# UWQuickstep/quickstep

Hardware: AMD Instinct MI355X
Metric: probe+aggregate rows/s at TPC-H SF100 (Q1,Q3) (higher is better)
Workload: dtype i32 keys / f64 sums

## Files before the change

### quickstep_amd/capi.py

```python
import ctypes as C
import os

import torch

from . import types as T

_HERE = os.path.dirname(os.path.abspath(__file__))
LIB_PATH = os.environ.get("QSX_LIB_PATH") or os.path.join(_HERE, "lib", "libqsx.so")


class QsxError(RuntimeError):
    def __init__(self, status, where):
        self.status = status
        msg = _lib.qsx_status_string(status).decode()
        detail = _lib.qsx_last_error().decode()
        super().__init__(f"{where}: {msg} ({status})" + (f" — {detail}" if detail and status in (T.ERR_HIP, T.ERR_COMM) else ""))


def _load():
    if not os.path.exists(LIB_PATH):
        raise ImportError(
            f"{LIB_PATH} is missing: build it with `python -c 'import __graft_entry__ as g; g.build()'` "
            "(or make -C quickstep_amd/csrc). There is no CPU fallback for the HIP execution kernel.")
    return C.CDLL(LIB_PATH)
# ... 1078 lines not shown
        _check(_lib.qsx_agg_state_export_bytes(self._h, C.byref(v), _stream(stream)), "qsx_agg_state_export_bytes")
        return v.value

    def export(self, device, stream=None):
        nbytes = self.export_bytes(stream)
        out = torch.empty(nbytes // 8, dtype=torch.int64, device=device)
        _check(_lib.qsx_agg_state_export(self._h, _ptr(out), nbytes, _stream(stream)), "qsx_agg_state_export")
        return out

    def image_layout(self):
        dense, header, per_col, ncols = C.c_int(), C.c_int64(), C.c_int64(), C.c_int()
        kinds = (C.c_int32 * 32)()
        _check(_lib.qsx_agg_state_image_layout(self._h, C.byref(dense), C.byref(header), C.byref(per_col), C.byref(ncols), kinds, 32),
               "qsx_agg_state_image_layout")
        return bool(dense.value), header.value, per_col.value, [int(kinds[i]) for i in range(ncols.value)]

    def import_merge(self, image, stream=None):
        _check(_lib.qsx_agg_state_import_merge(self._h, _ptr(image), image.numel() * image.element_size(), _stream(stream)),
               "qsx_agg_state_import_merge")

    def num_groups(self, stream=None):
        v = C.c_int64()
        _check(_lib.qsx_agg_num_groups(self._h, C.byref(v), _stream(stream)), "qsx_agg_num_groups")
        return v.value

    def finalize(self, device, partition=0, num_partitions=1, capacity=None, stream=None):
        cfg = self.config
        if capacity is None:
            capacity = max(self.num_groups(stream), 1)
        keys = []
        for k in range(cfg.num_keys):
            w = cfg.column_width[cfg.key_column[k]]
            dt = {1: torch.uint8, 2: torch.int16, 4: torch.int32, 8: torch.int64}[w]
            keys.append(torch.zeros(capacity, dtype=dt, device=device))
        vals, nulls = [], []
        for a in range(cfg.num_aggs):
            dt = getattr(torch, T.agg_output_dtype(cfg, a))
            vals.append(torch.zeros(capacity, dtype=dt, device=device))
            nulls.append(torch.zeros(capacity, dtype=torch.uint8, device=device))
        groups = torch.zeros(1, dtype=torch.int64, device=device)
        _check(_lib.qsx_agg_finalize(self._h, partition, num_partitions, _ptr_array(keys), _ptr_array(vals),
                                     _ptr_array(nulls), capacity, _ptr(groups), _stream(stream)), "qsx_agg_finalize")
        return keys, vals, nulls, groups


class LipFilter:
    def __init__(self, kind, cardinality, min_value=0, is_anti=False):
        h = C.c_void_p()
        _check(_lib.qsx_lip_filter_create(kind, cardinality, min_value, 1 if is_anti else 0, C.byref(h)),
               "qsx_lip_filter_create")
        self._h = h

    def close(self):
        if self._h is not None:
            _lib.qsx_lip_filter_destroy(self._h)
            self._h = None

    def __del__(self):
        try:
            self.close()
        except Exception:
            pass

    def build(self, keys, filter_bitmap=None, stream=None):
        _check(_lib.qsx_lip_build(self._h, qsx_type_of(keys), _ptr(keys), keys.numel(), _ptr(filter_bitmap),
                                  _stream(stream)), "qsx_lip_build")

    def build_from_table(self, table, num_new_keys=-1, stream=None):
        rc = _lib.qsx_lip_build_from_join_table(self._h, table._h, num_new_keys, _stream(stream))
        if rc == T.ERR_UNSUPPORTED:
            return False
        _check(rc, "qsx_lip_build_from_join_table")
        return True
# ... 168 lines not shown
```

### quickstep_amd/csrc/aggregate.hip

```cpp

#include "agg_common.hpp"
#include "agg_translate.hpp"
#include "agg_hash_update.hpp"
#include "agg_factored.hpp"
#include "agg_shapes.hpp"
#include "agg_stream.hpp"
#include "agg_family.hpp"
#include "agg_pieces.hpp"
#include "agg_jit.hpp"
#include "comm.hpp"
#include "partition.hpp"
#include "scan.hpp"

#include <atomic>
#include <cstdlib>
#include <map>
#include <mutex>
#include <shared_mutex>
#include <vector>

namespace qsx {

struct ColKinds {
  int kind[QSX_MAX_AGGS + 1];
// ... 48 lines not shown
    }
  }
}

__global__ __launch_bounds__(kABlock) void init_log_kernel(unsigned long long *__restrict__ log, int stride,
                                                          unsigned long long count, const unsigned int *__restrict__ count_dev,
                                                          unsigned int log_cap, ColKinds kinds) {
  if (count_dev != nullptr) count = *count_dev < log_cap ? *count_dev : log_cap;
  const unsigned long long words = count * stride;
  for (unsigned long long i = static_cast<unsigned long long>(blockIdx.x) * kABlock + threadIdx.x; i < words;
       i += static_cast<unsigned long long>(gridDim.x) * kABlock) {
    const int w = static_cast<int>(i % stride);
    log[i] = w == 0 ? kEmptyCode : static_cast<unsigned long long>(acc_identity(kinds.kind[w - 1]));
  }
}

__global__ __launch_bounds__(kABlock) void drain_log_kernel(const unsigned long long *__restrict__ records, unsigned int count,
                                                           int stride, int num_cols, ColKinds kinds, HashTableView g) {
  for (unsigned int r = blockIdx.x * kABlock + threadIdx.x; r < count; r += gridDim.x * kABlock) {
    const unsigned long long *rec = records + static_cast<unsigned long long>(r) * stride;
    const unsigned long long gs = global_find_or_insert(g, rec[0]);
    if (gs == ~0ull) continue;
    for (int col = 0; col < num_cols; ++col) global_add(g, col, gs, rec[1 + col], kinds.kind[col]);
  }
}

__global__ void publish_control_kernel(const unsigned long long *__restrict__ control, unsigned long long *host_slot,
                                       unsigned long long seq) {
  if (threadIdx.x != 0) return;
  __hip_atomic_store(&host_slot[0], control[0], __ATOMIC_RELAXED, __HIP_MEMORY_SCOPE_SYSTEM);
  __hip_atomic_store(&host_slot[1], control[3], __ATOMIC_RELAXED, __HIP_MEMORY_SCOPE_SYSTEM);
  __hip_atomic_store(&host_slot[2], control[1], __ATOMIC_RELAXED, __HIP_MEMORY_SCOPE_SYSTEM);
  __hip_atomic_store(&host_slot[3], seq, __ATOMIC_RELEASE, __HIP_MEMORY_SCOPE_SYSTEM);
}


__device__ __forceinline__ double avg_quotient(double s, double c) {
  const double q = s / c;
  if (!isfinite(q) || fabs(q) >= 2.2250738585072014e-308) return q;
  double best = q, best_r = fabs(fma(-q, c, s));
  const double around[2] = {nextafter(q, -INFINITY), nextafter(q, INFINITY)};
  for (const double x : around) {
    const double r = fabs(fma(-x, c, s));
    if (r < best_r || (r == best_r && (__double_as_longlong(x) & 1) == 0)) {
      best = x;
      best_r = r;
    }
  }
  return best;
}

__device__ __forceinline__ void write_values(const FinalizeDesc &f, const unsigned long long *states,
                                             unsigned long long col_stride, unsigned long long idx,
                                             int count_col, bool empty_group, long long out_row) {
  const long long cnt = count_col >= 0 ? static_cast<long long>(states[static_cast<unsigned long long>(count_col) * col_stride + idx]) : 0;
  for (int a = 0; a < f.num_aggs; ++a) {
    bool is_null = false;
    const bool has_nn = f.nn_col[a] >= 0;
    const long long seen = has_nn ? static_cast<long long>(states[static_cast<unsigned long long>(f.nn_col[a]) * col_stride + idx]) : cnt;
    if (f.fn[a] == QSX_AGG_COUNT_STAR) {
      static_cast<long long *>(f.out_vals[a])[out_row] = cnt;
    } else if (f.fn[a] == QSX_AGG_COUNT) {
      static_cast<long long *>(f.out_vals[a])[out_row] = seen;
    } else {
      const unsigned long long raw = states[static_cast<unsigned long long>(f.sum_col[a]) * col_stride + idx];
      if (f.fn[a] == QSX_AGG_SUM) {
// ... 35 lines not shown

__device__ __forceinline__ void write_keys_from_code(const FinalizeDesc &f, unsigned long long code, long long out_row,
                                                     const unsigned long long *states = nullptr, unsigned long long stride = 0,
                                                     unsigned long long slot = 0) {
  for (int k = 0; k < f.num_keys; ++k) {
    const unsigned long long v = group_key_word(f, code, states, stride, slot, f.key_word[k]) >> f.key_shift[k];
    switch (f.key_width[k]) {
      case 1: static_cast<uint8_t *>(f.out_keys[k])[out_row] = static_cast<uint8_t>(v); break;
      case 2: static_cast<uint16_t *>(f.out_keys[k])[out_row] = static_cast<uint16_t>(v); break;
      case 4: static_cast<uint32_t *>(f.out_keys[k])[out_row] = static_cast<uint32_t>(v); break;
      default: static_cast<unsigned long long *>(f.out_keys[k])[out_row] = v; break;
    }
  }
}

__device__ __forceinline__ unsigned long long reference_scalar_hash(int type, unsigned long long bits) {
  switch (type) {
    case QSX_INT: return bits & 0xFFFFFFFFull;
    case QSX_FLOAT: return (bits & 0xFFFFFFFFull) == 0x80000000ull ? 0ull : (bits & 0xFFFFFFFFull);
    case QSX_DOUBLE: return bits == 0x8000000000000000ull ? 0ull : bits;
    default: return bits;
  }
}
__device__ __forceinline__ unsigned long long reference_combine(unsigned long long a, unsigned long long b) {
  const unsigned long long kMul = 0x9ddfea08eb382d69ull;
  unsigned long long x = (a ^ b) * kMul;
  x ^= (x >> 47);
  unsigned long long y = (b ^ x) * kMul;
  y ^= (y >> 47);
  y *= kMul;
  return y;
}

__global__ __launch_bounds__(kABlock) void finalize_hash_kernel(HashTableView g, FinalizeDesc f,
                                                               int partition, int num_partitions,
                                                               int partition_by_hash, long long capacity,
                                                               unsigned long long *__restrict__ out_groups) {
  const unsigned long long stride = g.cap + 1;
  const unsigned long long total = g.cap + 1;
  const unsigned long long rounded = (total + kWave - 1) / kWave * kWave;
  for (unsigned long long i = static_cast<unsigned long long>(blockIdx.x) * kABlock + threadIdx.x;
       i < rounded; i += static_cast<unsigned long long>(gridDim.x) * kABlock) {
    bool emit = false;
    unsigned long long code = kEmptyCode;
    if (i < total) {
      code = i == g.cap ? kEmptyCode : g.keys[i];
      const unsigned long long cnt = g.states[i];
      emit = (i == g.cap) ? (cnt != 0) : (code != kEmptyCode);
      if (emit && partition_by_hash) {
        unsigned long long h = 0;
        for (int k = 0; k < f.num_keys; ++k) {
          unsigned long long bits = group_key_word(f, code, g.states, stride, i, f.key_word[k]) >> f.key_shift[k];
          if (f.key_width[k] < 8) bits &= (1ull << (8 * f.key_width[k])) - 1;
          const unsigned long long hk = reference_scalar_hash(f.key_type[k], bits);
          h = k == 0 ? hk : reference_combine(h, hk);
        }
        emit = static_cast<int>(h % static_cast<unsigned long long>(num_partitions)) == partition;
      }
    }
    const uint64_t m = __ballot(emit);
    if (m == 0) continue;
    const int leader = __ffsll(static_cast<long long>(m)) - 1;
    unsigned long long base = 0;
    if (lane_id() == leader) base = atomicAdd(out_groups, static_cast<unsigned long long>(__popcll(m)));
    base = __shfl(base, leader, kWave);
    if (!emit) continue;
    const long long out_row = static_cast<long long>(base) + rank_below(m);
    if (out_row >= capacity) continue;
    write_keys_from_code(f, code, out_row, g.states, stride, i);
    write_values(f, g.states, stride, i, 0, false, out_row);
  }
}

constexpr int kExprRows = 2;
struct ExprProgram {
  const void *cols[QSX_MAX_COLUMNS];
  int types[QSX_MAX_COLUMNS];
  int num_instrs;
  DevInstr instrs[QSX_MAX_INSTRS];
  double consts[QSX_MAX_CONSTS];
  DevOperand result;
};
static_assert(sizeof(ExprProgram) % 4 == 0, "store_struct_kernel copies words");
__device__ __forceinline__ void expr_operand(const ExprProgram &p, const DevOperand &o, const Temps<kExprRows> &t, const int64_t (&row)[kExprRows],
                                             double (&out)[kExprRows]) {
  switch (o.kind) {
    case QSX_OPD_COLUMN: {
      const void *col = as_global(p.cols[o.index]);
#pragma unroll
      for (int v = 0; v < kExprRows; ++v) {
        switch (p.types[o.index]) {
          case QSX_INT: out[v] = static_cast<double>(static_cast<const int32_t *>(col)[row[v]]); break;
          case QSX_LONG: out[v] = static_cast<double>(static_cast<const long long *>(col)[row[v]]); break;
          case QSX_FLOAT: out[v] = static_cast<double>(static_cast<const float *>(col)[row[v]]); break;
          default: out[v] = static_cast<const double *>(col)[row[v]]; break;
        }
      }
      break;
    }
    case QSX_OPD_CONST:
#pragma unroll
      for (int v = 0; v < kExprRows; ++v) out[v] = p.consts[o.index];
      break;
    default:
// ... 1505 lines not shown
  }
  if (err == hipSuccess && fill_identities(st, nullptr) != QSX_OK) err = hipErrorUnknown;
  if (err == hipSuccess) err = hipDeviceSynchronize();
  if (err != hipSuccess) {
    set_last_error("qsx_agg_state_create", err);
    (void)device_free(st->image); (void)device_free(st->control); (void)device_free(st->tile_counts); (void)device_free(st->tile_offsets);
    (void)device_free(st->log);
    (void)device_free(st->dir_entries); (void)device_free(st->dir_codes); (void)device_free(st->dir_words); (void)device_free(st->dir_ngids);
    published_slots().give(st->published);
    delete st;
    return err == hipErrorOutOfMemory ? QSX_ERR_OUT_OF_MEMORY : QSX_ERR_HIP;
  }
  *out = st;
  return QSX_OK;
}

int qsx_agg_state_destroy(qsx_agg_state_t *st) {
  if (st == nullptr) return QSX_OK;
  (void)synchronize_owner_device(st->image);
  (void)device_free_idle(st->image);
  (void)device_free_idle(st->control);
  (void)device_free_idle(st->tile_counts);
  (void)device_free_idle(st->tile_offsets);
  (void)device_free_idle(st->log);
  (void)device_free_idle(st->dir_entries);
  (void)device_free_idle(st->dir_codes);
  (void)device_free_idle(st->dir_words);
  (void)device_free_idle(st->dir_ngids);
  published_slots().give(st->published);
  delete st;
  return QSX_OK;
}

int qsx_agg_state_clear(qsx_agg_state_t *st, qsx_stream_t stream) {
  QSX_REQUIRE_DEVICE();
  if (st == nullptr) return QSX_ERR_INVALID_ARGUMENT;
  hipStream_t s = as_stream(stream);
  std::unique_lock<std::shared_mutex> lock(st->table_mutex);
  if (st->growable) {
    int rc = init_log(st, st->log, 0, reinterpret_cast<const unsigned int *>(st->control + 3), s);
    if (rc != QSX_OK) return rc;
    __atomic_store_n(&st->published[0], 0ull, __ATOMIC_RELEASE);
    __atomic_store_n(&st->published[1], 0ull, __ATOMIC_RELEASE);
  }
  if (st->dir_gids != 0) {
    QSX_HIP_TRY(hipMemsetAsync(st->dir_entries, 0xFF, st->dir_cap * 8 * st->dir_entry_words, s));
    QSX_HIP_TRY(hipMemsetAsync(st->dir_ngids, 0, 16, s));
  }
  if (st->dense) {
    QSX_HIP_TRY(hipMemsetAsync(st->image, 0, st->image_bytes, s));
  } else {
    QSX_HIP_TRY(hipMemsetAsync(st->image, 0xFF, sizeof(unsigned long long) * (st->cap + 1), s));
    QSX_HIP_TRY(hipMemsetAsync(st->image + (st->cap + 1), 0,
                               sizeof(unsigned long long) * (st->cap + 1) * st->num_cols, s));
  }
  QSX_HIP_TRY(hipMemsetAsync(st->control, 0, 8 * sizeof(unsigned long long), s));
  return fill_identities(st, s);
}

static void decide_dense_families(qsx_agg_state *st, const void *key_col, int64_t rows, hipStream_t s) {
  if (st->dense_families.load() != 0) return;
  DevConfig dev = st->dev;
  plan_tile(dev, st->used_columns, kDirBlock, false);
  const DenseLdsGeometry geo = dense_lds_geometry(st->config.num_entries, st->num_sums, static_cast<size_t>(dev.tile_bytes), true);
  if (geo.entries == 0 || geo.ranges == 1) {
    st->dense_families.store(1);
    return;
  }
  const int key_col_index = st->dev.key_column[0];
  const int sample = static_cast<int>(std::min<int64_t>(rows, 256 * 1024));
  if (key_col == nullptr || st->dev.code_width[key_col_index] != 0 || sample < 4096) {
// ... 1569 lines not shown
    switch (o.kind) {
      case QSX_OPD_COLUMN: return types[o.index] == QSX_INT;
      case QSX_OPD_CONST: return consts[o.index] >= INT32_MIN && consts[o.index] <= INT32_MAX;
      default: return temp_is_int[o.index];
    }
  };
  for (int k = 0; k < num_instrs; ++k) {
    const qsx_expr_instr_t &in = instrs[k];
    if (in.op < QSX_EX_ADD || in.op > QSX_EX_IDIV || in.dst < 0 || in.dst >= QSX_MAX_TEMPS || !valid(in.a) || !valid(in.b)) {
      return QSX_ERR_INVALID_ARGUMENT;
    }
    prog.instrs[k].op = in.op & 3;
    prog.instrs[k].dst = in.dst;
    prog.instrs[k].a = DevOperand{in.a.kind, in.a.index};
    prog.instrs[k].b = DevOperand{in.b.kind, in.b.index};
    prog.narrow[k] = is_int(in.a) && is_int(in.b) ? 1 : 0;
    temp_is_int[in.dst] = prog.narrow[k] != 0;
    defined |= 1 << in.dst;
  }
  if (!valid(result)) return QSX_ERR_INVALID_ARGUMENT;
  prog.result = DevOperand{result.kind, result.index};
  for (int k = 0; k < QSX_MAX_CONSTS; ++k) prog.consts[k] = consts != nullptr ? consts[k] : 0;
  if (n == 0) return QSX_OK;
  hipStream_t s = as_stream(stream);
  IntExprProgram *slot = device_slot<IntExprProgram>(s);
  if (slot == nullptr) return QSX_ERR_OUT_OF_MEMORY;
  hipLaunchKernelGGL(store_struct_kernel<IntExprProgram>, dim3(1), dim3(64), 0, s, prog, slot);
  QSX_CHECK_LAUNCH();
  hipLaunchKernelGGL(eval_expression_long_kernel, dim3(grid_for(n, kABlock * 4)), dim3(kABlock), 0, s, slot, n, out_width, out_dev);
  QSX_CHECK_LAUNCH();
  return QSX_OK;
}

int qsx_agg_finalize(qsx_agg_state_t *st, int partition, int num_partitions, void *const *out_key_cols,
                     void *const *out_val_cols, uint8_t *const *out_null_cols, int64_t capacity,
                     int64_t *out_groups_dev, qsx_stream_t stream) {
  QSX_REQUIRE_DEVICE();
  if (st == nullptr || out_groups_dev == nullptr || num_partitions < 1 || partition < 0 ||
      partition >= num_partitions || capacity < 0 || out_val_cols == nullptr) {
    return QSX_ERR_INVALID_ARGUMENT;
  }
  hipStream_t s = as_stream(stream);
  int rc = settle(st, s);
  if (rc != QSX_OK) return rc;
  std::shared_lock<std::shared_mutex> lock(st->table_mutex);
  FinalizeDesc f = st->fin;
  for (int k = 0; k < f.num_keys; ++k) {
    if (out_key_cols == nullptr || out_key_cols[k] == nullptr) return QSX_ERR_INVALID_ARGUMENT;
    f.out_keys[k] = out_key_cols[k];
  }
  for (int a = 0; a < f.num_aggs; ++a) {
    f.out_vals[a] = out_val_cols[a];
    f.out_nulls[a] = out_null_cols != nullptr ? out_null_cols[a] : nullptr;
  }
  unsigned long long *out_groups = reinterpret_cast<unsigned long long *>(out_groups_dev);
  QSX_HIP_TRY(hipMemsetAsync(out_groups_dev, 0, sizeof(int64_t), s));
  f.collision = reinterpret_cast<int *>(st->control + 4);
  switch (st->config.strategy) {
    case QSX_AGG_SINGLE_STATE:
      if (partition != 0) return QSX_OK;
      if (capacity < 1) return QSX_ERR_CAPACITY;
      hipLaunchKernelGGL(finalize_single_kernel, dim3(1), dim3(64), 0, s, st->hash_view(), f, out_groups);
      break;
    case QSX_AGG_COMPACT_KEY:
      if (partition != 0) return QSX_OK;
      hipLaunchKernelGGL(finalize_hash_kernel, dim3(grid_for(st->cap + 1, kABlock)), dim3(kABlock), 0, s,
                         st->hash_view(), f, 0, 1, 0, static_cast<long long>(capacity), out_groups);
      break;
    case QSX_AGG_GENERIC:
      hipLaunchKernelGGL(finalize_hash_kernel, dim3(grid_for(st->cap + 1, kABlock)), dim3(kABlock), 0, s,
                         st->hash_view(), f, partition, num_partitions, 1, static_cast<long long>(capacity),
                         out_groups);
      break;
    default: {
      const DenseRange range = dense_partition_range(st->config.num_entries, num_partitions, partition);
      const long long begin = range.begin, end = range.end;
      if (begin >= end) return QSX_OK;
      const long long first_word = range.first_word;
      const long long num_words = range.last_word - first_word;
      const long long num_tiles = (num_words + kDenseTileWords - 1) / kDenseTileWords;
      const DenseView d = st->dense_view();
      CallScratch scratch(s);
      const size_t counts_bytes = sizeof(int32_t) * static_cast<size_t>(num_tiles + 1), offsets_bytes = sizeof(int64_t) * static_cast<size_t>(num_tiles + 2);
      const int rc_scratch = scratch.reserve(CallScratch::padded(counts_bytes) + CallScratch::padded(offsets_bytes));
      if (rc_scratch != QSX_OK) return rc_scratch;
      int32_t *tile_counts = static_cast<int32_t *>(scratch.take(counts_bytes));
      int64_t *tile_offsets = static_cast<int64_t *>(scratch.take(offsets_bytes));
      hipLaunchKernelGGL(dense_tile_count_kernel, dim3(grid_for(num_tiles, kABlock / kWave)), dim3(kABlock), 0, s,
                         d.exist, first_word, num_words, begin, end, num_tiles, tile_counts);
      QSX_CHECK_LAUNCH();
      hipLaunchKernelGGL(tile_scan_kernel, dim3(1), dim3(1024), 0, s, tile_counts,
                         static_cast<int64_t>(num_tiles), tile_offsets, out_groups_dev);
      QSX_CHECK_LAUNCH();
      hipLaunchKernelGGL(finalize_dense_kernel, dim3(grid_for(num_tiles, kABlock / kWave)), dim3(kABlock), 0, s,
                         d, f, first_word, num_words, begin, end, num_tiles, tile_offsets,
                         static_cast<long long>(capacity));
      break;
    }
  }
  QSX_CHECK_LAUNCH();
  if (f.wide_words != 0) {
    hipLaunchKernelGGL(report_collision_kernel, dim3(1), dim3(64), 0, s, f.collision, out_groups);
    QSX_CHECK_LAUNCH();
  }
  return QSX_OK;
}

}
```

### quickstep_amd/csrc/join.hip

```cpp

#include "common.hpp"
#include "join_dense.hpp"
#include "join_lds.hpp"
#include "scan.hpp"

#include <atomic>
#include <cstdlib>
#include <vector>
#include <mutex>
#include <shared_mutex>
#include <type_traits>

namespace qsx {

constexpr int kJBlock = 256;
constexpr uint64_t kEmpty64 = ~0ull;
constexpr uint32_t kEmptyTid = 0xFFFFFFFFu;

struct alignas(16) LongEntry {
  int64_t key;
  uint32_t tid;
  uint32_t pad;
};

// ... 219 lines not shown
  for (int64_t i = static_cast<int64_t>(blockIdx.x) * kJBlock + threadIdx.x; i < cap;
       i += static_cast<int64_t>(gridDim.x) * kJBlock) {
    if (is_long) {
      const LongEntry e = static_cast<const LongEntry *>(src.slots)[i];
      if (e.tid != kEmptyTid) insert_entry(dst, e.key, e.tid);
    } else {
      const uint64_t e = static_cast<const uint64_t *>(src.slots)[i];
      if (e != kEmpty64) {
        insert_entry(dst, static_cast<int32_t>(static_cast<uint32_t>(e)), static_cast<uint32_t>(e >> 32));
      }
    }
  }
}

__global__ __launch_bounds__(kJBlock) void compact_build_kernel(TableView t, uint32_t *__restrict__ cslots, unsigned char *__restrict__ cfp) {
  const uint64_t s = static_cast<uint64_t>(blockIdx.x) * kJBlock + threadIdx.x;
  if (s >= t.num_slots()) return;
  unsigned char f = 0;
  uint32_t packed = 0xFFFFFFFFu;
  if (t.fp[s] != 0) {
    const uint64_t e = static_cast<const uint64_t *>(t.slots)[s];
    const CompactId id = compact_id(static_cast<int32_t>(static_cast<uint32_t>(e)), t.buckets);
    if (id.bucket == static_cast<uint32_t>(s / kBucketSlots)) {
      f = static_cast<unsigned char>(id.fp);
      packed = (id.low << 24) | (static_cast<uint32_t>(e >> 32) & 0xFFFFFFu);
    } else {
      f = 0xFFu;
    }
  }
  cfp[s] = f;
  cslots[s] = packed;
}

__global__ __launch_bounds__(kJBlock) void dense_pack_kernel(const uint32_t *__restrict__ head, uint64_t range, unsigned char *__restrict__ head3) {
  for (uint64_t i = static_cast<uint64_t>(blockIdx.x) * kJBlock + threadIdx.x; i < range; i += static_cast<uint64_t>(gridDim.x) * kJBlock) {
    const uint32_t w = head[i];
    const uint32_t packed = (w & 0x7FFFFFu) | ((w & kChainBit) >> 8);
    head3[i * 3] = static_cast<unsigned char>(packed);
    head3[i * 3 + 1] = static_cast<unsigned char>(packed >> 8);
    head3[i * 3 + 2] = static_cast<unsigned char>(packed >> 16);
  }
}

__global__ __launch_bounds__(kJBlock) void dense_build_from_slots_kernel(int is_long, TableView src, DenseTableView d) {
  const int64_t cap = static_cast<int64_t>(src.num_slots());
  for (int64_t i = static_cast<int64_t>(blockIdx.x) * kJBlock + threadIdx.x; i < cap;
       i += static_cast<int64_t>(gridDim.x) * kJBlock) {
    int64_t key;
    uint32_t tid;
    if (is_long) {
      const LongEntry e = static_cast<const LongEntry *>(src.slots)[i];
      if (e.tid == kEmptyTid) continue;
      key = e.key;
      tid = e.tid;
    } else {
      const uint64_t e = static_cast<const uint64_t *>(src.slots)[i];
      if (e == kEmpty64) continue;
      key = static_cast<int32_t>(static_cast<uint32_t>(e));
      tid = static_cast<uint32_t>(e >> 32);
    }
    const uint64_t idx = dense_index(d, key);
    if (idx == ~0ull) {
      atomicExch(d.error, 1);
      continue;
    }
    const uint32_t old = atomicCAS(&d.head[idx], 0u, tid + 1u);
    if (old != 0u) {
      const unsigned int e = atomicAdd(d.ov_count, 1u);
      if (e >= d.ov_capacity) {
        atomicExch(d.error, 2);
        continue;
      }
      d.ov[e].x = tid;
      d.ov[e].y = atomicExch(&d.head[idx], kChainBit | e);
// ... 754 lines not shown
  return join_key_pack_blocks_impl(ncols, types, num_blocks, block_rows, block_cols, block_code_widths, block_dictionaries, out_dev, out_exact, stream);
}

static int destroy_table(qsx_join_table_t *t, bool wait_for_device) {
  if (t == nullptr) return QSX_OK;
  if (wait_for_device) {
    (void)synchronize_owner_device(t->slots != nullptr ? static_cast<const void *>(t->slots) : static_cast<const void *>(t->head));
  }
  if (t->shadow != nullptr) (void)destroy_table(t->shadow, wait_for_device);
  (void)device_free_idle(t->slots);
  (void)device_free_idle(t->head);
  (void)device_free_idle(t->head3);
  (void)device_free_idle(t->compact);
  (void)device_free_idle(t->cover);
  if (t->pack_event != nullptr) (void)hipEventDestroy(t->pack_event);
  if (t->seal_event != nullptr) (void)hipEventDestroy(t->seal_event);
  for (auto &m : t->marks) {
    if (m.second != nullptr) (void)hipEventDestroy(m.second);
  }
  if (t->control_host != nullptr) (void)hipHostFree(t->control_host);
  (void)device_free_idle(t->ov);
  (void)device_free_idle(t->entries_dev);
  delete t;
  return QSX_OK;
}
int qsx_join_table_destroy(qsx_join_table_t *t) { return destroy_table(t, true); }
int qsx_join_table_release(qsx_join_table_t *t) { return destroy_table(t, false); }

int qsx_join_table_clear(qsx_join_table_t *t, qsx_stream_t stream) {
  QSX_REQUIRE_DEVICE();
  if (t == nullptr) return QSX_ERR_INVALID_ARGUMENT;
  std::unique_lock<std::shared_mutex> lock(t->mutex);
  if (t->dense) {
    QSX_HIP_TRY(hipMemsetAsync(t->head, 0, t->range * sizeof(uint32_t), as_stream(stream)));
  } else {
    const int rc_fill = fill_empty(t, t->slots, t->capacity, as_stream(stream));
    if (rc_fill != QSX_OK) return rc_fill;
  }
  const int rc_control = reset_control_words(t->entries_dev, as_stream(stream));
  if (rc_control != QSX_OK) return rc_control;
  t->reserved = 0;
  t->max_tid.store(-1);
  t->seal_state.store(0);
  t->scanned.store(false);
  drop_cover(t);
  mark_stream(t, as_stream(stream));
  return QSX_OK;
}

int qsx_join_table_size(qsx_join_table_t *t, int64_t *out_entries, qsx_stream_t stream) {
  QSX_REQUIRE_DEVICE();
  if (t == nullptr || out_entries == nullptr) return QSX_ERR_INVALID_ARGUMENT;
  unsigned long long v[kControlWords] = {0, 0, 0, 0, 0, 0};
  const int rc_words = copy_control_words(t->entries_dev, as_stream(stream), v);
  if (rc_words != QSX_OK) return rc_words;
  *out_entries = static_cast<int64_t>(v[0]);
  if (t->dense && static_cast<int>(v[3] & 0xFFFFFFFFu) != 0) return QSX_ERR_INVALID_ARGUMENT;
  return QSX_OK;
}

int qsx_join_build(qsx_join_table_t *t, const void *keys_dev, int64_t n, int32_t base_tid,
                   const uint64_t *filter_dev, qsx_stream_t stream) {
  QSX_REQUIRE_DEVICE();
  if (t == nullptr || n < 0 || base_tid < 0) return QSX_ERR_INVALID_ARGUMENT;
  if (n == 0) return QSX_OK;
  if (keys_dev == nullptr) return QSX_ERR_INVALID_ARGUMENT;
  if (static_cast<int64_t>(base_tid) + n > INT32_MAX) return QSX_ERR_INVALID_ARGUMENT;
  int rc = ensure_room(t, n);
  if (rc != QSX_OK) return rc;
  t->seal_state.store(0);
  t->scanned.store(false);
  drop_cover(t);
  for (int64_t seen = t->max_tid.load(); seen < base_tid + n - 1 && !t->max_tid.compare_exchange_weak(seen, base_tid + n - 1);) {}
// ... 109 lines not shown
int qsx_join_build_blocks_coded(qsx_join_table_t *t, int64_t num_blocks, const int64_t *block_rows, const void *const *block_keys,
                                const qsx_key_coding_t *coding, const int32_t *block_base_tids, const uint64_t *const *block_filters,
                                qsx_stream_t stream) {
  return join_build_blocks_impl(t, num_blocks, block_rows, block_keys, block_base_tids, block_filters, coding, stream);
}

}

static std::atomic<long long> g_compact_probes{0};
extern "C" long long qsx_debug_join_compact_probes(void) { return g_compact_probes.load(std::memory_order_relaxed); }
static bool lds_tables_enabled() {
  const char *e = getenv("QSX_JOIN_LDS");
  return e == nullptr || e[0] != '0';
}

static bool dense_two_pass(const uint64_t *filter) {
  const char *e = getenv("QSX_JOIN_TWO_PASS");
  if (e != nullptr && e[0] != '\0') return e[0] != '0';
  return filter != nullptr;
}

static void drop_cover(qsx_join_table *t) {
  std::lock_guard<std::mutex> lock(t->cover_mutex);
  t->cover_state = 0;
  t->cover_sig.clear();
}

constexpr int64_t kAdaptiveMinRows = 1 << 16;
static bool adaptive_enabled() {
  const char *e = getenv("QSX_JOIN_ADAPTIVE");
  return e == nullptr || e[0] != '0';
}

static void sealed_pack(qsx_join_table *t, hipStream_t stream) {
  auto behind_the_pack = [&]() {
    if (t->pack_stream != stream && t->pack_event != nullptr && hipEventQuery(t->pack_event) != hipSuccess) {
      (void)hipGetLastError();
      (void)hipStreamWaitEvent(stream, t->pack_event, 0);
    }
  };
  int state = t->seal_state.load(std::memory_order_acquire);
  if (state == 2) {
    behind_the_pack();
    return;
  }
  if (state != 0 || !adaptive_enabled()) return;
  const uint64_t bytes4 = t->range * 4, bytes3 = t->range * 3;
  if (bytes4 <= (13ull << 18) || bytes3 > (36ull << 20) / 10 || t->max_tid.load() >= (1 << 23) - 2 || t->reserved >= (1 << 23) - 1) {
    return;
  }
  std::lock_guard<std::mutex> lock(t->seal_mutex);
  state = t->seal_state.load(std::memory_order_acquire);
  if (state != 0) {
    if (state == 2) behind_the_pack();
    return;
  }
  if (t->head3 == nullptr && device_malloc(&t->head3, static_cast<size_t>(bytes3) + 4) != hipSuccess) {
    (void)hipGetLastError();
    t->head3 = nullptr;
    t->seal_state.store(1, std::memory_order_release);
    return;
  }
  if (t->pack_event == nullptr && hipEventCreateWithFlags(&t->pack_event, hipEventDisableTiming) != hipSuccess) {
    (void)hipGetLastError();
    t->pack_event = nullptr;
    t->seal_state.store(1, std::memory_order_release);
    return;
  }
  hipLaunchKernelGGL(dense_pack_kernel, dim3(grid_for(static_cast<int64_t>(t->range), kJBlock * 4)), dim3(kJBlock), 0, stream, t->head, t->range,
                     t->head3);
  if (hipGetLastError() != hipSuccess || hipEventRecord(t->pack_event, stream) != hipSuccess) {
    (void)hipGetLastError();
    (void)hipStreamSynchronize(stream);
    t->seal_state.store(1, std::memory_order_release);
    return;
  }
  t->pack_stream = stream;
  t->seal_state.store(2, std::memory_order_release);
}

static bool compact_enabled() {
  const char *e = getenv("QSX_JOIN_COMPACT");
  return e == nullptr || e[0] != '0';
}
static bool compact_possible(const qsx_join_table *t) {
  const uint64_t buckets = t->capacity / kBucketSlots;
  return compact_enabled() && t->key_type == QSX_INT && buckets >= kCompactMinBuckets && buckets <= 0xFFFFFFFFull && t->max_tid.load() < (1 << 24);
}
static bool seal_compact(qsx_join_table *t, bool duplicate_keys, hipStream_t stream) {
  if (!compact_possible(t) || duplicate_keys) return false;
  if (t->compact_capacity != t->capacity) {
    (void)device_free(t->compact);
    t->compact = nullptr;
    t->compact_capacity = 0;
    if (device_malloc(&t->compact, static_cast<size_t>(t->capacity) * 5 + 16) != hipSuccess) {
      (void)hipGetLastError();
      t->compact = nullptr;
      return false;
    }
    t->compact_capacity = t->capacity;
  }
  hipLaunchKernelGGL(compact_build_kernel, dim3(static_cast<unsigned>((t->capacity + kJBlock - 1) / kJBlock)), dim3(kJBlock), 0, stream, t->view(),
                     static_cast<uint32_t *>(t->compact), static_cast<unsigned char *>(t->compact) + t->capacity * 4);
  if (hipGetLastError() != hipSuccess) return false;
  return true;
}

static bool seal_verify_enabled() {
  const char *e = getenv("QSX_JOIN_SEAL_VERIFY");
  return e != nullptr && e[0] == '1';
}
// ... 160 lines not shown
    const int sub = kLds ? kLdsSub : kLdsSubGlobal, per_cu = kLds ? 1 : 2;
    const int64_t units = (tiles + sub - 1) / sub;
    const int grid = static_cast<int>(units < static_cast<int64_t>(per_cu) * kCUs ? units : static_cast<int64_t>(per_cu) * kCUs);
    hipLaunchKernelGGL(kernel, dim3(grid), dim3(kLdsBlock), table_bytes, stream, t->dense_view(), static_cast<const KeyT *>(keys), n, probe_base_tid,
                       filter, out_probe, out_build, capacity, count, out_bitmap, anti, runs_dev, lips);
    QSX_CHECK_LAUNCH();
    return QSX_OK;
  };
  return t->key_type == QSX_INT ? launch(int32_t{}) : launch(int64_t{});
}

static bool one_pass_enabled() {
  const char *e = getenv("QSX_JOIN_ONE_PASS");
  return e == nullptr || e[0] != '0';
}

template <int MODE, bool kRuns = false>
static int launch_probe(qsx_join_table_t *t, const void *keys, int64_t n, int32_t probe_base_tid,
                        const uint64_t *filter, int32_t *out_probe, int32_t *out_build,
                        int64_t capacity, int64_t *out_count, uint64_t *out_bitmap, int anti,
                        hipStream_t stream, const long long *runs_dev = nullptr, int64_t run_tiles = 0) {
  static_assert(kDenseTile == kProbeTile, "one run table serves both table kinds");
  if (!t->dense && n != 0) {
    qsx_join_table *shadow = sealed_shadow(t, stream, n);
    if (shadow != nullptr) {
      return launch_probe<MODE, kRuns>(shadow, keys, n, probe_base_tid, filter, out_probe, out_build, capacity, out_count, out_bitmap,
                                       anti, stream, runs_dev, run_tiles);
    }
    if (!t->scanned.load(std::memory_order_acquire)) {
      set_last_error("the scan in front of a hashed table's first probe could not be issued", hipErrorUnknown);
      return QSX_ERR_HIP;
    }
  }
  if (out_count != nullptr) QSX_HIP_TRY(hipMemsetAsync(out_count, 0, sizeof(int64_t), stream));
  if (n == 0) return QSX_OK;
  if (t->dense) sealed_pack(t, stream);
  std::shared_lock<std::shared_mutex> lock(t->mutex);
  if (t->dense) {
    const int64_t tiles = kRuns ? run_tiles : (n + kDenseTile - 1) / kDenseTile;
    const int64_t limit = 8 * kCUs;
    const int dgrid = static_cast<int>(tiles < limit ? tiles : limit);
    unsigned long long *dcount = reinterpret_cast<unsigned long long *>(out_count);
    if constexpr (MODE == 0 || MODE == 1 || MODE == 2) {
      const bool two_pass = MODE == 0 && dense_two_pass(filter);
      if (!two_pass && lds_tables_enabled() && t->range <= static_cast<uint64_t>(kLdsDenseMaxWords) && n >= 32 * static_cast<int64_t>(t->range) &&
          n >= (1 << 18)) {
        return launch_lds_dense_probe<MODE, kRuns>(t, keys, n, probe_base_tid, filter, out_probe, out_build, capacity, dcount, out_bitmap, anti,
                                                   stream, runs_dev, tiles);
      }
    }
    if constexpr (MODE == 0) {
      if (dense_two_pass(filter) && one_pass_enabled() && n >= (1 << 20)) {
        return launch_lds_dense_probe<0, kRuns, false>(t, keys, n, probe_base_tid, filter, out_probe, out_build, capacity, dcount, out_bitmap, anti,
                                                       stream, runs_dev, tiles);
      }
    }
    if (MODE == 0 && dense_two_pass(filter)) {
      const int64_t units = tiles * (kDBlock / kWave);
      CallScratch scratch(stream);
      const size_t bytes_counts = static_cast<size_t>(units) * 4, bytes_offsets = static_cast<size_t>(units + 1) * 8,
                   bytes_scan = scan_workspace_words(units) * 8;
      const int rc_scratch = scratch.reserve(CallScratch::padded(bytes_counts) + CallScratch::padded(bytes_offsets) + CallScratch::padded(bytes_scan));
      if (rc_scratch != QSX_OK) return rc_scratch;
      int32_t *unit_counts = static_cast<int32_t *>(scratch.take(bytes_counts));
      int64_t *unit_offsets = static_cast<int64_t *>(scratch.take(bytes_offsets)), *scan_ws = static_cast<int64_t *>(scratch.take(bytes_scan));
      if (t->key_type == QSX_INT) {
        hipLaunchKernelGGL((dense_probe_kernel<int32_t, 3, kRuns>), dim3(dgrid), dim3(kDBlock), 0, stream, t->dense_view(),
                           static_cast<const int32_t *>(keys), n, probe_base_tid, filter, out_probe, out_build, capacity,
                           dcount, out_bitmap, anti, unit_counts, unit_offsets, runs_dev);
// ... 597 lines not shown
```

Baseline: 193.6 billion.

## Fold memsets and control readbacks into fewer kernel launches across agg and join paths

Replaces zero-initialised output allocations with empty ones and zeroes only the unused tail rows on device. Adds a single-block finalize kernel for small hash tables that counts groups in shared memory and publishes the control words to pinned host memory, avoiding a separate memset and device-to-host copy. Merges the aggregation state clear into one kernel and the dense join clear with its control reset, and folds the probe count reset into the pack kernel. This cuts launch and API overhead per call, at the cost of more complex code and new paths for correctness bugs (tail zeroing, control handoff ordering).

```diff
diff --git a/quickstep_amd/capi.py b/quickstep_amd/capi.py
--- a/quickstep_amd/capi.py
+++ b/quickstep_amd/capi.py
@@ -1134,13 +1134,13 @@
         for k in range(cfg.num_keys):
             w = cfg.column_width[cfg.key_column[k]]
             dt = {1: torch.uint8, 2: torch.int16, 4: torch.int32, 8: torch.int64}[w]
-            keys.append(torch.zeros(capacity, dtype=dt, device=device))
+            keys.append(torch.empty(capacity, dtype=dt, device=device))
         vals, nulls = [], []
         for a in range(cfg.num_aggs):
             dt = getattr(torch, T.agg_output_dtype(cfg, a))
-            vals.append(torch.zeros(capacity, dtype=dt, device=device))
-            nulls.append(torch.zeros(capacity, dtype=torch.uint8, device=device))
-        groups = torch.zeros(1, dtype=torch.int64, device=device)
+            vals.append(torch.empty(capacity, dtype=dt, device=device))
+            nulls.append(torch.empty(capacity, dtype=torch.uint8, device=device))
+        groups = torch.empty(1, dtype=torch.int64, device=device)
         _check(_lib.qsx_agg_finalize(self._h, partition, num_partitions, _ptr_array(keys), _ptr_array(vals),
                                      _ptr_array(nulls), capacity, _ptr(groups), _stream(stream)), "qsx_agg_finalize")
         return keys, vals, nulls, groups
diff --git a/quickstep_amd/csrc/aggregate.hip b/quickstep_amd/csrc/aggregate.hip
--- a/quickstep_amd/csrc/aggregate.hip
+++ b/quickstep_amd/csrc/aggregate.hip
@@ -104,6 +104,48 @@
   __hip_atomic_store(&host_slot[1], control[3], __ATOMIC_RELAXED, __HIP_MEMORY_SCOPE_SYSTEM);
   __hip_atomic_store(&host_slot[2], control[1], __ATOMIC_RELAXED, __HIP_MEMORY_SCOPE_SYSTEM);
   __hip_atomic_store(&host_slot[3], seq, __ATOMIC_RELEASE, __HIP_MEMORY_SCOPE_SYSTEM);
+}
+
+struct ClearDesc {
+  unsigned long long *image;
+  unsigned long long slots;
+  int num_cols;
+  ColKinds kinds;
+  unsigned long long *dir_entries;
+  unsigned long long dir_words;
+  unsigned int *dir_ngids;
+  unsigned long long *log;
+  int log_stride;
+  unsigned int log_cap;
+  unsigned long long *control;
+};
+__global__ __launch_bounds__(kABlock) void clear_hash_state_kernel(ClearDesc c) {
+  const unsigned long long image_words = c.slots * static_cast<unsigned long long>(c.num_cols + 1);
+  const unsigned long long total = image_words + (c.dir_entries != nullptr ? c.dir_words : 0ull);
+  for (unsigned long long i = static_cast<unsigned long long>(blockIdx.x) * kABlock + threadIdx.x; i < total;
+       i += static_cast<unsigned long long>(gridDim.x) * kABlock) {
+    if (i < c.slots) {
+      c.image[i] = kEmptyCode;
+    } else if (i < image_words) {
+      c.image[i] = static_cast<unsigned long long>(acc_identity(c.kinds.kind[static_cast<int>(i / c.slots) - 1]));
+    } else {
+      c.dir_entries[i - image_words] = ~0ull;
+    }
+  }
+  if (blockIdx.x != 0) return;
+  if (c.dir_entries != nullptr && threadIdx.x < 4) c.dir_ngids[threadIdx.x] = 0u;
+  unsigned long long records = 0;
+  if (c.log != nullptr) {
+    const unsigned int left = *reinterpret_cast<const unsigned int *>(c.control + 3);
+    records = left < c.log_cap ? left : c.log_cap;
+  }
+  __syncthreads();
+  const unsigned long long log_words = records * static_cast<unsigned long long>(c.log_stride);
+  for (unsigned long long i = threadIdx.x; i < log_words; i += kABlock) {
+    const int w = static_cast<int>(i % c.log_stride);
+    c.log[i] = w == 0 ? kEmptyCode : static_cast<unsigned long long>(acc_identity(c.kinds.kind[w - 1]));
+  }
+  if (threadIdx.x < 8) c.control[threadIdx.x] = 0ull;
 }
 
 
@@ -205,32 +247,72 @@
   return y;
 }
 
+__device__ __forceinline__ int out_value_width(const FinalizeDesc &f, int a) {
+  const bool typed = f.fn[a] == QSX_AGG_MIN || f.fn[a] == QSX_AGG_MAX;
+  return typed && (f.val_type[a] == QSX_INT || f.val_type[a] == QSX_FLOAT) ? 4 : 8;
+}
+__device__ __forceinline__ void zero_output_row(const FinalizeDesc &f, long long out_row) {
+  for (int k = 0; k < f.num_keys; ++k) {
+    switch (f.key_width[k]) {
+      case 1: static_cast<uint8_t *>(f.out_keys[k])[out_row] = 0; break;
+      case 2: static_cast<uint16_t *>(f.out_keys[k])[out_row] = 0; break;
+      case 4: static_cast<uint32_t *>(f.out_keys[k])[out_row] = 0; break;
+      default: static_cast<unsigned long long *>(f.out_keys[k])[out_row] = 0; break;
+    }
+  }
+  for (int a = 0; a < f.num_aggs; ++a) {
+    if (out_value_width(f, a) == 4) static_cast<uint32_t *>(f.out_vals[a])[out_row] = 0;
+    else static_cast<unsigned long long *>(f.out_vals[a])[out_row] = 0;
+    if (f.out_nulls[a] != nullptr) f.out_nulls[a][out_row] = 0;
+  }
+}
+__global__ __launch_bounds__(kABlock) void finalize_tail_kernel(FinalizeDesc f, const unsigned long long *__restrict__ groups,
+                                                               long long capacity) {
+  const unsigned long long found = *groups;
+  const long long first = found < static_cast<unsigned long long>(capacity) ? static_cast<long long>(found) : capacity;
+  for (long long row = first + static_cast<long long>(blockIdx.x) * kABlock + threadIdx.x; row < capacity;
+       row += static_cast<long long>(gridDim.x) * kABlock) {
+    zero_output_row(f, row);
+  }
+}
+
+__device__ __forceinline__ bool slot_emits(const HashTableView &g, const FinalizeDesc &f, unsigned long long i, int partition,
+                                           int num_partitions, int partition_by_hash, unsigned long long *code_out) {
+  const unsigned long long stride = g.cap + 1;
+  const unsigned long long code = i == g.cap ? kEmptyCode : g.keys[i];
+  *code_out = code;
+  const unsigned long long cnt = g.states[i];
+  bool emit = (i == g.cap) ? (cnt != 0) : (code != kEmptyCode);
+  if (emit && partition_by_hash) {
+    unsigned long long h = 0;
+    for (int k = 0; k < f.num_keys; ++k) {
+      unsigned long long bits = group_key_word(f, code, g.states, stride, i, f.key_word[k]) >> f.key_shift[k];
+      if (f.key_width[k] < 8) bits &= (1ull << (8 * f.key_width[k])) - 1;
+      const unsigned long long hk = reference_scalar_hash(f.key_type[k], bits);
+      h = k == 0 ? hk : reference_combine(h, hk);
+    }
+    emit = static_cast<int>(h % static_cast<unsigned long long>(num_partitions)) == partition;
+  }
+  return emit;
+}
+
+__device__ __forceinline__ void hand_control_words(const unsigned long long *control, unsigned long long *control_out) {
+  for (int w = 0; w < 4; ++w) __hip_atomic_store(&control_out[w], control[w], __ATOMIC_RELAXED, __HIP_MEMORY_SCOPE_SYSTEM);
+}
+
 __global__ __launch_bounds__(kABlock) void finalize_hash_kernel(HashTableView g, FinalizeDesc f,
                                                                int partition, int num_partitions,
                                                                int partition_by_hash, long long capacity,
-                                                               unsigned long long *__restrict__ out_groups) {
+                                                               unsigned long long *__restrict__ out_groups,
+                                                               unsigned long long *control_out) {
+  if (control_out != nullptr && blockIdx.x == 0 && threadIdx.x == 0) hand_control_words(g.ngroups, control_out);
   const unsigned long long stride = g.cap + 1;
   const unsigned long long total = g.cap + 1;
   const unsigned long long rounded = (total + kWave - 1) / kWave * kWave;
   for (unsigned long long i = static_cast<unsigned long long>(blockIdx.x) * kABlock + threadIdx.x;
        i < rounded; i += static_cast<unsigned long long>(gridDim.x) * kABlock) {
-    bool emit = false;
     unsigned long long code = kEmptyCode;
-    if (i < total) {
-      code = i == g.cap ? kEmptyCode : g.keys[i];
-      const unsigned long long cnt = g.states[i];
-      emit = (i == g.cap) ? (cnt != 0) : (code != kEmptyCode);
-      if (emit && partition_by_hash) {
-        unsigned long long h = 0;
-        for (int k = 0; k < f.num_keys; ++k) {
-          unsigned long long bits = group_key_word(f, code, g.states, stride, i, f.key_word[k]) >> f.key_shift[k];
-          if (f.key_width[k] < 8) bits &= (1ull << (8 * f.key_width[k])) - 1;
-          const unsigned long long hk = reference_scalar_hash(f.key_type[k], bits);
-          h = k == 0 ? hk : reference_combine(h, hk);
-        }
-        emit = static_cast<int>(h % static_cast<unsigned long long>(num_partitions)) == partition;
-      }
-    }
+    const bool emit = i < total && slot_emits(g, f, i, partition, num_partitions, partition_by_hash, &code);
     const uint64_t m = __ballot(emit);
     if (m == 0) continue;
     const int leader = __ffsll(static_cast<long long>(m)) - 1;
@@ -243,6 +325,41 @@
     write_keys_from_code(f, code, out_row, g.states, stride, i);
     write_values(f, g.states, stride, i, 0, false, out_row);
   }
+}
+
+constexpr int kFinalizeBlockThreads = 1024;
+__global__ __launch_bounds__(kFinalizeBlockThreads) void finalize_hash_block_kernel(HashTableView g, FinalizeDesc f,
+                                                                     int partition, int num_partitions,
+                                                                     int partition_by_hash, long long capacity,
+                                                                     unsigned long long *__restrict__ out_groups,
+                                                                     unsigned long long *control_out) {
+  __shared__ unsigned long long s_groups;
+  if (threadIdx.x == 0) s_groups = 0;
+  if (control_out != nullptr && threadIdx.x == 0) hand_control_words(g.ngroups, control_out);
+  __syncthreads();
+  const unsigned long long stride = g.cap + 1;
+  const unsigned long long total = g.cap + 1;
+  const unsigned long long rounded = (total + kWave - 1) / kWave * kWave;
+  for (unsigned long long i = threadIdx.x; i < rounded; i += kFinalizeBlockThreads) {
+    unsigned long long code = kEmptyCode;
+    const bool emit = i < total && slot_emits(g, f, i, partition, num_partitions, partition_by_hash, &code);
+    const uint64_t m = __ballot(emit);
+    if (m == 0) continue;
+    const int leader = __ffsll(static_cast<long long>(m)) - 1;
+    unsigned long long base = 0;
+    if (lane_id() == leader) base = atomicAdd(&s_groups, static_cast<unsigned long long>(__popcll(m)));
+    base = __shfl(base, leader, kWave);
+    if (!emit) continue;
+    const long long out_row = static_cast<long long>(base) + rank_below(m);
+    if (out_row >= capacity) continue;
+    write_keys_from_code(f, code, out_row, g.states, stride, i);
+    write_values(f, g.states, stride, i, 0, false, out_row);
+  }
+  __syncthreads();
+  const unsigned long long found = s_groups;
+  if (threadIdx.x == 0) *out_groups = found;
+  const long long first = found < static_cast<unsigned long long>(capacity) ? static_cast<long long>(found) : capacity;
+  for (long long row = first + threadIdx.x; row < capacity; row += kFinalizeBlockThreads) zero_output_row(f, row);
 }
 
 constexpr int kExprRows = 2;
@@ -1814,11 +1931,45 @@
   return QSX_OK;
 }
 
+}
+
+static unsigned long long clear_one_kernel_max_words() {
+  const char *e = getenv("QSX_AGG_CLEAR_ONE_KERNEL_WORDS");
+  return e != nullptr ? static_cast<unsigned long long>(atoll(e)) : 1ull << 25;
+}
+
+extern "C" {
+
 int qsx_agg_state_clear(qsx_agg_state_t *st, qsx_stream_t stream) {
   QSX_REQUIRE_DEVICE();
   if (st == nullptr) return QSX_ERR_INVALID_ARGUMENT;
   hipStream_t s = as_stream(stream);
   std::unique_lock<std::shared_mutex> lock(st->table_mutex);
+  if (!st->dense) {
+    const unsigned long long dir_words = st->dir_gids != 0 ? st->dir_cap * st->dir_entry_words : 0ull;
+    const unsigned long long words = (st->cap + 1) * (st->num_cols + 1) + dir_words;
+    if (words <= clear_one_kernel_max_words()) {
+      ClearDesc c{};
+      c.image = st->image;
+      c.slots = st->cap + 1;
+      c.num_cols = st->num_cols;
+      c.kinds = st->col_kinds;
+      c.dir_entries = st->dir_gids != 0 ? st->dir_entries : nullptr;
+      c.dir_words = dir_words;
+      c.dir_ngids = st->dir_ngids;
+      c.log = st->growable ? st->log : nullptr;
+      c.log_stride = st->num_cols + 1;
+      c.log_cap = kLogRecords;
+      c.control = st->control;
+      hipLaunchKernelGGL(clear_hash_state_kernel, dim3(grid_for(static_cast<int64_t>(words), kABlock * 4)), dim3(kABlock), 0, s, c);
+      QSX_CHECK_LAUNCH();
+      if (st->growable) {
+        __atomic_store_n(&st->published[0], 0ull, __ATOMIC_RELEASE);
+        __atomic_store_n(&st->published[1], 0ull, __ATOMIC_RELEASE);
+      }
+      return QSX_OK;
+    }
+  }
   if (st->growable) {
     int rc = init_log(st, st->log, 0, reinterpret_cast<const unsigned int *>(st->control + 3), s);
     if (rc != QSX_OK) return rc;
@@ -3454,50 +3605,58 @@
   return QSX_OK;
 }
 
-int qsx_agg_finalize(qsx_agg_state_t *st, int partition, int num_partitions, void *const *out_key_cols,
-                     void *const *out_val_cols, uint8_t *const *out_null_cols, int64_t capacity,
-                     int64_t *out_groups_dev, qsx_stream_t stream) {
-  QSX_REQUIRE_DEVICE();
-  if (st == nullptr || out_groups_dev == nullptr || num_partitions < 1 || partition < 0 ||
-      partition >= num_partitions || capacity < 0 || out_val_cols == nullptr) {
-    return QSX_ERR_INVALID_ARGUMENT;
-  }
-  hipStream_t s = as_stream(stream);
-  int rc = settle(st, s);
-  if (rc != QSX_OK) return rc;
-  std::shared_lock<std::shared_mutex> lock(st->table_mutex);
-  FinalizeDesc f = st->fin;
-  for (int k = 0; k < f.num_keys; ++k) {
-    if (out_key_cols == nullptr || out_key_cols[k] == nullptr) return QSX_ERR_INVALID_ARGUMENT;
-    f.out_keys[k] = out_key_cols[k];
-  }
-  for (int a = 0; a < f.num_aggs; ++a) {
-    f.out_vals[a] = out_val_cols[a];
-    f.out_nulls[a] = out_null_cols != nullptr ? out_null_cols[a] : nullptr;
-  }
+}
+
+constexpr unsigned long long kFinalizeBlockSlots = 8192;
+constexpr int64_t kFinalizeBlockRows = 8192;
+
+struct CallControlWords {
+  unsigned long long *host = published_slots().take();
+  unsigned long long *dev = nullptr;
+  CallControlWords() {
+    if (host != nullptr && hipHostGetDevicePointer(reinterpret_cast<void **>(&dev), host, 0) != hipSuccess) {
+      (void)hipGetLastError();
+      dev = nullptr;
+    }
+  }
+  ~CallControlWords() { published_slots().give(host); }
+  CallControlWords(const CallControlWords &) = delete;
+  CallControlWords &operator=(const CallControlWords &) = delete;
+};
+
+static int launch_finalize(qsx_agg_state *st, const FinalizeDesc &f, int partition, int num_partitions, int64_t capacity,
+                           int64_t *out_groups_dev, hipStream_t s, unsigned long long *control_out, bool *handed) {
+  *handed = false;
   unsigned long long *out_groups = reinterpret_cast<unsigned long long *>(out_groups_dev);
-  QSX_HIP_TRY(hipMemsetAsync(out_groups_dev, 0, sizeof(int64_t), s));
-  f.collision = reinterpret_cast<int *>(st->control + 4);
+  bool tail_done = false;
+  bool emits = true;
   switch (st->config.strategy) {
     case QSX_AGG_SINGLE_STATE:
-      if (partition != 0) return QSX_OK;
+      if (partition != 0) { emits = false; break; }
       if (capacity < 1) return QSX_ERR_CAPACITY;
       hipLaunchKernelGGL(finalize_single_kernel, dim3(1), dim3(64), 0, s, st->hash_view(), f, out_groups);
       break;
     case QSX_AGG_COMPACT_KEY:
-      if (partition != 0) return QSX_OK;
-      hipLaunchKernelGGL(finalize_hash_kernel, dim3(grid_for(st->cap + 1, kABlock)), dim3(kABlock), 0, s,
-                         st->hash_view(), f, 0, 1, 0, static_cast<long long>(capacity), out_groups);
+    case QSX_AGG_GENERIC: {
+      const bool generic = st->config.strategy == QSX_AGG_GENERIC;
+      if (!generic && partition != 0) { emits = false; break; }
+      if (st->cap + 1 <= kFinalizeBlockSlots && capacity <= kFinalizeBlockRows) {
+        hipLaunchKernelGGL(finalize_hash_block_kernel, dim3(1), dim3(kFinalizeBlockThreads), 0, s, st->hash_view(), f, generic ? partition : 0,
+                           generic ? num_partitions : 1, generic ? 1 : 0, static_cast<long long>(capacity), out_groups, control_out);
+        tail_done = true;
+      } else {
+        QSX_HIP_TRY(hipMemsetAsync(out_groups_dev, 0, sizeof(int64_t), s));
+        hipLaunchKernelGGL(finalize_hash_kernel, dim3(grid_for(st->cap + 1, kABlock)), dim3(kABlock), 0, s, st->hash_view(), f,
+                           generic ? partition : 0, generic ? num_partitions : 1, generic ? 1 : 0, static_cast<long long>(capacity),
+                           out_groups, control_out);
+      }
+      *handed = control_out != nullptr;
       break;
-    case QSX_AGG_GENERIC:
-      hipLaunchKernelGGL(finalize_hash_kernel, dim3(grid_for(st->cap + 1, kABlock)), dim3(kABlock), 0, s,
-                         st->hash_view(), f, partition, num_partitions, 1, static_cast<long long>(capacity),
-                         out_groups);
-      break;
+    }
     default: {
       const DenseRange range = dense_partition_range(st->config.num_entries, num_partitions, partition);
       const long long begin = range.begin, end = range.end;
-      if (begin >= end) return QSX_OK;
+      if (begin >= end) { emits = false; break; }
       const long long first_word = range.first_word;
       const long long num_words = range.last_word - first_word;
       const long long num_tiles = (num_words + kDenseTileWords - 1) / kDenseTileWords;
@@ -3520,12 +3679,71 @@
       break;
     }
   }
-  QSX_CHECK_LAUNCH();
-  if (f.wide_words != 0) {
+  if (emits) QSX_CHECK_LAUNCH();
+  else QSX_HIP_TRY(hipMemsetAsync(out_groups_dev, 0, sizeof(int64_t), s));
+  if (!tail_done && capacity > 0) {
+    hipLaunchKernelGGL(finalize_tail_kernel, dim3(grid_for(capacity, kABlock)), dim3(kABlock), 0, s, f, out_groups,
+                       static_cast<long long>(capacity));
+    QSX_CHECK_LAUNCH();
+  }
+  if (emits && f.wide_words != 0) {
     hipLaunchKernelGGL(report_collision_kernel, dim3(1), dim3(64), 0, s, f.collision, out_groups);
     QSX_CHECK_LAUNCH();
   }
   return QSX_OK;
 }
 
-}
+extern "C" {
+
+int qsx_agg_finalize(qsx_agg_state_t *st, int partition, int num_partitions, void *const *out_key_cols,
+                     void *const *out_val_cols, uint8_t *const *out_null_cols, int64_t capacity,
+                     int64_t *out_groups_dev, qsx_stream_t stream) {
+  QSX_REQUIRE_DEVICE();
+  if (st == nullptr || out_groups_dev == nullptr || num_partitions < 1 || partition < 0 ||
+      partition >= num_partitions || capacity < 0 || out_val_cols == nullptr) {
+    return QSX_ERR_INVALID_ARGUMENT;
+  }
+  hipStream_t s = as_stream(stream);
+  FinalizeDesc f = st->fin;
+  bool valid = true;
+  for (int k = 0; k < f.num_keys; ++k) {
+    valid = valid && out_key_cols != nullptr && out_key_cols[k] != nullptr;
+    if (valid) f.out_keys[k] = out_key_cols[k];
+  }
+  for (int a = 0; a < f.num_aggs; ++a) {
+    f.out_vals[a] = out_val_cols[a];
+    f.out_nulls[a] = out_null_cols != nullptr ? out_null_cols[a] : nullptr;
+  }
+  f.collision = reinterpret_cast<int *>(st->control + 4);
+  CallControlWords words;
+  int launched = QSX_ERR_INVALID_ARGUMENT;
+  unsigned long long control[4] = {0, 0, 0, 0};
+  bool handed = false;
+  {
+    std::shared_lock<std::shared_mutex> lock(st->table_mutex);
+    if (valid) launched = launch_finalize(st, f, partition, num_partitions, capacity, out_groups_dev, s, words.dev, &handed);
+    if (launched != QSX_OK) handed = false;
+    if (!handed) QSX_HIP_TRY(hipMemcpyAsync(control, st->control, sizeof(control), hipMemcpyDeviceToHost, s));
+  }
+  QSX_HIP_TRY(hipStreamSynchronize(s));
+  if (handed) {
+    for (int w = 0; w < 4; ++w) control[w] = __atomic_load_n(&words.host[w], __ATOMIC_ACQUIRE);
+  }
+  if (static_cast<int>(control[1] & 0xFFFFFFFFu) != 0) {
+    return st->dense ? QSX_ERR_INVALID_ARGUMENT : QSX_ERR_TOO_MANY_GROUPS;
+  }
+  if (st->growable && ((control[3] & 0xFFFFFFFFull) != 0 || control[0] * 4 > st->cap)) {
+    {
+      std::unique_lock<std::shared_mutex> lock(st->table_mutex);
+      const int rc = grow_and_drain(st);
+      if (rc != QSX_OK) return rc;
+    }
+    if (launched != QSX_OK) return launched;
+    std::shared_lock<std::shared_mutex> lock(st->table_mutex);
+    launched = launch_finalize(st, f, partition, num_partitions, capacity, out_groups_dev, s, nullptr, &handed);
+    if (launched == QSX_OK) QSX_HIP_TRY(hipStreamSynchronize(s));
+  }
+  return launched;
+}
+
+}
diff --git a/quickstep_amd/csrc/join.hip b/quickstep_amd/csrc/join.hip
--- a/quickstep_amd/csrc/join.hip
+++ b/quickstep_amd/csrc/join.hip
@@ -275,7 +275,9 @@
   cslots[s] = packed;
 }
 
-__global__ __launch_bounds__(kJBlock) void dense_pack_kernel(const uint32_t *__restrict__ head, uint64_t range, unsigned char *__restrict__ head3) {
+__global__ __launch_bounds__(kJBlock) void dense_pack_kernel(const uint32_t *__restrict__ head, uint64_t range, unsigned char *__restrict__ head3,
+                                                             unsigned long long *count_word) {
+  if (count_word != nullptr && blockIdx.x == 0 && threadIdx.x == 0) *count_word = 0ull;
   for (uint64_t i = static_cast<uint64_t>(blockIdx.x) * kJBlock + threadIdx.x; i < range; i += static_cast<uint64_t>(gridDim.x) * kJBlock) {
     const uint32_t w = head[i];
     const uint32_t packed = (w & 0x7FFFFFu) | ((w & kChainBit) >> 8);
@@ -283,6 +285,18 @@
     head3[i * 3 + 1] = static_cast<unsigned char>(packed >> 8);
     head3[i * 3 + 2] = static_cast<unsigned char>(packed >> 16);
   }
+}
+
+__global__ __launch_bounds__(kJBlock) void dense_clear_kernel(uint32_t *__restrict__ head, uint64_t range, unsigned long long *__restrict__ control,
+                                                              int control_words) {
+  const uint64_t quads = range / 4;
+  uint4 *head4 = reinterpret_cast<uint4 *>(head);
+  for (uint64_t i = static_cast<uint64_t>(blockIdx.x) * kJBlock + threadIdx.x; i < quads; i += static_cast<uint64_t>(gridDim.x) * kJBlock) {
+    head4[i] = make_uint4(0u, 0u, 0u, 0u);
+  }
+  if (blockIdx.x != 0) return;
+  if (threadIdx.x < range - quads * 4) head[quads * 4 + threadIdx.x] = 0u;
+  for (int w = threadIdx.x; w < control_words; w += kJBlock) control[w] = 0ull;
 }
 
 __global__ __launch_bounds__(kJBlock) void dense_build_from_slots_kernel(int is_long, TableView src, DenseTableView d) {
@@ -1103,13 +1117,15 @@
   if (t == nullptr) return QSX_ERR_INVALID_ARGUMENT;
   std::unique_lock<std::shared_mutex> lock(t->mutex);
   if (t->dense) {
-    QSX_HIP_TRY(hipMemsetAsync(t->head, 0, t->range * sizeof(uint32_t), as_stream(stream)));
+    hipLaunchKernelGGL(dense_clear_kernel, dim3(grid_for(static_cast<int64_t>(t->range / 4), kJBlock * 4)), dim3(kJBlock), 0, as_stream(stream),
+                       t->head, t->range, t->entries_dev, static_cast<int>(kControlBytes / sizeof(unsigned long long)));
+    QSX_CHECK_LAUNCH();
   } else {
     const int rc_fill = fill_empty(t, t->slots, t->capacity, as_stream(stream));
     if (rc_fill != QSX_OK) return rc_fill;
-  }
-  const int rc_control = reset_control_words(t->entries_dev, as_stream(stream));
-  if (rc_control != QSX_OK) return rc_control;
+    const int rc_control = reset_control_words(t->entries_dev, as_stream(stream));
+    if (rc_control != QSX_OK) return rc_control;
+  }
   t->reserved = 0;
   t->max_tid.store(-1);
   t->seal_state.store(0);
@@ -1285,7 +1301,7 @@
   return e == nullptr || e[0] != '0';
 }
 
-static void sealed_pack(qsx_join_table *t, hipStream_t stream) {
+static bool sealed_pack(qsx_join_table *t, hipStream_t stream, unsigned long long *count_word = nullptr) {
   auto behind_the_pack = [&]() {
     if (t->pack_stream != stream && t->pack_event != nullptr && hipEventQuery(t->pack_event) != hipSuccess) {
       (void)hipGetLastError();
@@ -1295,41 +1311,42 @@
   int state = t->seal_state.load(std::memory_order_acquire);
   if (state == 2) {
     behind_the_pack();
-    return;
-  }
-  if (state != 0 || !adaptive_enabled()) return;
+    return false;
+  }
+  if (state != 0 || !adaptive_enabled()) return false;
   const uint64_t bytes4 = t->range * 4, bytes3 = t->range * 3;
   if (bytes4 <= (13ull << 18) || bytes3 > (36ull << 20) / 10 || t->max_tid.load() >= (1 << 23) - 2 || t->reserved >= (1 << 23) - 1) {
-    return;
+    return false;
   }
   std::lock_guard<std::mutex> lock(t->seal_mutex);
   state = t->seal_state.load(std::memory_order_acquire);
   if (state != 0) {
     if (state == 2) behind_the_pack();
-    return;
+    return false;
   }
   if (t->head3 == nullptr && device_malloc(&t->head3, static_cast<size_t>(bytes3) + 4) != hipSuccess) {
     (void)hipGetLastError();
     t->head3 = nullptr;
     t->seal_state.store(1, std::memory_order_release);
-    return;
+    return false;
   }
   if (t->pack_event == nullptr && hipEventCreateWithFlags(&t->pack_event, hipEventDisableTiming) != hipSuccess) {
     (void)hipGetLastError();
     t->pack_event = nullptr;
     t->seal_state.store(1, std::memory_order_release);
-    return;
+    return false;
   }
   hipLaunchKernelGGL(dense_pack_kernel, dim3(grid_for(static_cast<int64_t>(t->range), kJBlock * 4)), dim3(kJBlock), 0, stream, t->head, t->range,
-                     t->head3);
+                     t->head3, count_word);
   if (hipGetLastError() != hipSuccess || hipEventRecord(t->pack_event, stream) != hipSuccess) {
     (void)hipGetLastError();
     (void)hipStreamSynchronize(stream);
     t->seal_state.store(1, std::memory_order_release);
-    return;
+    return false;
   }
   t->pack_stream = stream;
   t->seal_state.store(2, std::memory_order_release);
+  return count_word != nullptr;
 }
 
 static bool compact_enabled() {
@@ -1556,9 +1573,9 @@
       return QSX_ERR_HIP;
     }
   }
-  if (out_count != nullptr) QSX_HIP_TRY(hipMemsetAsync(out_count, 0, sizeof(int64_t), stream));
+  const bool zeroed = n != 0 && t->dense && sealed_pack(t, stream, reinterpret_cast<unsigned long long *>(out_count));
+  if (out_count != nullptr && !zeroed) QSX_HIP_TRY(hipMemsetAsync(out_count, 0, sizeof(int64_t), stream));
   if (n == 0) return QSX_OK;
-  if (t->dense) sealed_pack(t, stream);
   std::shared_lock<std::shared_mutex> lock(t->mutex);
   if (t->dense) {
     const int64_t tiles = kRuns ? run_tiles : (n + kDenseTile - 1) / kDenseTile;
```

New measurement: 196.7 billion, median of 6. 1.02x the previous value.
